# 3dhumangan/3DHumanGAN

Measured on NVIDIA H100. Metric: images_per_sec_G_fwd_512x512, higher is better.
Workload: dtype f32 (bf16x3 split on wgmma, fp32 accumulate)

## Files before the change

### 3dhumangan_b200/csrc/synth.cu

```cuda
#include "common.cuh"
#include "wgmma.cuh"

namespace hg {

constexpr int kC = 256;
constexpr int kSynThreads = 384;
constexpr int kSynStages = 2;
constexpr int kASlots = 2;
constexpr int kXSlots = 5;
constexpr int kXs = 3;
constexpr int kSs = 2;
constexpr uint32_t kAChunk = 128 * 128;
constexpr uint32_t kBStage = 256 * 128;
constexpr uint32_t kXSlice = 32 * 128 * 4;

struct SpadeArgs {
  const float* x;
  long x_bstride;
  const float* mod;
  const float* scsh;
  const float* p_lr;
  long p_stride;
  const float* p_bias;
  const uint8_t* wgb;
  const float* bgb;
  const uint8_t* wimg;
  const float* bias;
  const float* skip;
  long skip_bstride;
  float* out;
  double* stats;
  const float* rgb_w;
  const float* rgb_b;
  const float* rgb_in;
  float* rgb_out;
  int B, HW, Hg, Wg, Rh, Rw;
  int nkc;
  int xC;
  const float* x2;
  float slope;
  int cout;
  int out_pm;
  int act;
  const float* ascale;
  const float* rk_v;
  int rk_n;
  const float* mod2;
};

struct SynSmem {
  uint8_t* a_hi;
  uint8_t* a_lo;
  uint8_t* b_st;
  float* x_st;
  int xs_n, ss_n;
  float* tab_g1;
  float* tab_g0;
  float* tab_bias;
  float* tab_rgbw;
  float* tab_bgb;
  float* tab_as;
  float* st_sum;
  float* st_sq;
  uint64_t* bars;
};

template <bool kPixel>
__device__ __forceinline__ SynSmem carve(uint8_t* raw) {
  constexpr int kA = kPixel ? 3 : kASlots, kX = kPixel ? 3 : kXSlots;
  uint8_t* s = reinterpret_cast<uint8_t*>((reinterpret_cast<uintptr_t>(raw) + 1023) & ~uintptr_t(1023));
  SynSmem m;
  m.a_hi = s;
  m.a_lo = s + kA * kAChunk;
  m.b_st = s + 2 * kA * kAChunk;
  m.x_st = reinterpret_cast<float*>(m.b_st + kSynStages * kBStage);
  m.xs_n = kPixel ? 2 : kXs;
  m.ss_n = kPixel ? 1 : kSs;
  float* f = m.x_st + kX * (kXSlice / 4);
  m.tab_g1 = f; f += kC;
  m.tab_g0 = f; f += kC;
  m.tab_bias = f; f += kC;
  m.tab_rgbw = f; f += 3 * kC;
  m.tab_bgb = f; f += 512;
  m.tab_as = f; f += kC;
  m.st_sum = f; f += kC;
  m.st_sq = f; f += kC;
  m.bars = reinterpret_cast<uint64_t*>(f);
  return m;
}
constexpr uint32_t kSynSmemBytes = 2 * kASlots * kAChunk + kSynStages * kBStage + kXSlots * kXSlice +
                                   (kC * 9 + 512) * 4 + 24 * 8 + 1024;
constexpr uint32_t kPixSmemBytes = 2 * 3 * kAChunk + kSynStages * kBStage + 3 * kXSlice + (kC * 9 + 512) * 4 + 24 * 8 + 1024;
static_assert(kSynSmemBytes <= 232448 && kPixSmemBytes <= 232448, "shared memory budget");

enum { B_FULL = 0 , B_EMPTY = 2 , X_FULL = 4 , X_EMPTY = 12  };

__device__ __forceinline__ void rows_barrier() { named_barrier(1, 256); }

__device__ __forceinline__ float lrelu02(float v) { return v > 0.f ? v : 0.2f * v; }

__device__ __forceinline__ float reduce_2pi(float t) {
  const float y = t * 0.15915494309189535f;
  const float k = (y + 12582912.f) - 12582912.f;
  float r = fmaf(-k, 6.2831854820251465f, t);
  return fmaf(-k, -1.7484555314695172e-07f, r);
}
__device__ __forceinline__ float sin_red(float t) { return __sinf(reduce_2pi(t)); }
__device__ __forceinline__ float cos_red(float t) { return __cosf(reduce_2pi(t)); }
__device__ __forceinline__ float2 reduce_2pi2(float2 t) {
  const float2 y = fmul2(t, make_float2(0.15915494309189535f, 0.15915494309189535f));
  const float2 k = fadd2(fadd2(y, make_float2(12582912.f, 12582912.f)), make_float2(-12582912.f, -12582912.f));
  const float2 r = ffma2(k, make_float2(-6.2831854820251465f, -6.2831854820251465f), t);
  return ffma2(k, make_float2(1.7484555314695172e-07f, 1.7484555314695172e-07f), r);
}
__device__ __forceinline__ float2 sin_red2(float2 t) { const float2 r = reduce_2pi2(t); return make_float2(__sinf(r.x), __sinf(r.y)); }
__device__ __forceinline__ float2 cos_red2(float2 t) { const float2 r = reduce_2pi2(t); return make_float2(__cosf(r.x), __cosf(r.y)); }

struct TileMap {
  int T, first, stride, count;
  __device__ __forceinline__ void get(int it, int& b, int& ti) const {
    const int tile = first + it * stride;
    b = tile / T;
    ti = tile - b * T;
  }
};

__device__ __forceinline__ void init_common(const SpadeArgs& a, const SynSmem& m) {
  for (int i = threadIdx.x; i < kC; i += blockDim.x) {
    m.tab_bias[i] = a.bias[i];
    m.st_sum[i] = 0.f;
    m.st_sq[i] = 0.f;
  }
  if (a.rgb_w)
    for (int i = threadIdx.x; i < 3 * kC; i += blockDim.x) m.tab_rgbw[i] = a.rgb_w[i];
  if (threadIdx.x == 0) {
    for (int i = 0; i < kSynStages; ++i) {
      mbar_init(m.bars + B_FULL + i, 1);
      mbar_init(m.bars + B_EMPTY + i, 2);
    }
    for (int i = 0; i < m.xs_n + m.ss_n; ++i) {
      mbar_init(m.bars + X_FULL + i, 1);
      mbar_init(m.bars + X_EMPTY + i, 8);
    }
    fence_mbar_init();
  }
  __syncthreads();
}

template <int kPasses>
__device__ __forceinline__ void weight_producer_loop(const SynSmem& m, const uint8_t* img, int nstages, int num_my_tiles) {
  uint32_t st = 0, ph = 0;
  for (int t = 0; t < num_my_tiles; ++t)
    for (int s = 0; s < nstages; ++s) {
      if (kPasses == 1 && (s & 1)) continue;
      mbar_wait_backoff(m.bars + B_EMPTY + st, ph ^ 1);
      mbar_arrive_expect_tx(m.bars + B_FULL + st, kBStage);
      bulk_g2s(m.b_st + st * kBStage, img + static_cast<size_t>(s) * kBStage, kBStage, m.bars + B_FULL + st);
      if (++st == kSynStages) { st = 0; ph ^= 1; }
    }
}

struct Pipe {
  uint32_t st = 0, ph = 0, prev = ~0u;
};
template <int N, int kPasses>
__device__ __forceinline__ void pipe_chunk(const SynSmem& m, Pipe& p, float (&d)[N / 2], uint32_t a_hi, uint32_t a_lo, bool accumulate,
                                           int t) {
#pragma unroll
  for (int part = 0; part < (kPasses == 3 ? 2 : 1); ++part) {
    mbar_wait(m.bars + B_FULL + p.st, p.ph);
    acc_fence(d);
    wgmma_fence();
    const uint32_t bt = smem_u32(m.b_st + p.st * kBStage);
    if (part == 0) {
      wg_k64<N>(d, a_hi, bt, accumulate);
      if (kPasses == 3) wg_k64<N>(d, a_lo, bt, true);
    } else {
      wg_k64<N>(d, a_hi, bt, true);
    }
    wgmma_commit();
    wgmma_wait<1>();
    acc_fence(d);
    if (p.prev != ~0u && t == 0) mbar_arrive(m.bars + B_EMPTY + p.prev);
    p.prev = p.st;
    if (++p.st == kSynStages) { p.st = 0; p.ph ^= 1; }
  }
}
template <int N>
__device__ __forceinline__ void pipe_drain(const SynSmem& m, Pipe& p, float (&d)[N / 2], int t) {
  wgmma_wait<0>();
  acc_fence(d);
  if (p.prev != ~0u && t == 0) mbar_arrive(m.bars + B_EMPTY + p.prev);
  p.prev = ~0u;
}

__device__ __forceinline__ void ring_emit(const SynSmem& m, uint32_t& g, int base, int slots, const float* src) {
  const uint32_t slot = base + g % slots;
  mbar_wait_backoff(m.bars + X_EMPTY + slot, ((g / slots) & 1) ^ 1);
  mbar_arrive_expect_tx(m.bars + X_FULL + slot, kXSlice);
  bulk_g2s(m.x_st + slot * (kXSlice / 4), src, kXSlice, m.bars + X_FULL + slot);
  ++g;
}
__device__ __forceinline__ void x_producer_loop(const SpadeArgs& a, const SynSmem& m, const TileMap& tm) {
  uint32_t g = 0;
  for (int it = 0; it < tm.count; ++it) {
    int b, ti;
    tm.get(it, b, ti);
    const int per_src = a.xC / 32;
    const float* base = a.x + static_cast<long>(b) * a.x_bstride + static_cast<long>(ti) * a.xC * 128;
    const float* base2 = a.x2 ? a.x2 + (static_cast<long>(b) * tm.T + ti) * a.xC * 128 : nullptr;
    for (int j = 0; j < 2 * a.nkc; ++j)
      ring_emit(m, g, 0, m.xs_n, (j < per_src ? base : base2 - per_src * 32 * 128) + j * 32 * 128);
  }
}
__device__ __forceinline__ void skip_producer_loop(const SpadeArgs& a, const SynSmem& m, const TileMap& tm) {
  if (!a.skip) return;
  uint32_t g = 0;
  for (int it = 0; it < tm.count; ++it) {
    int b, ti;
    tm.get(it, b, ti);
    const float* base = a.skip + static_cast<long>(b) * a.skip_bstride + static_cast<long>(ti) * a.cout * 128;
    for (int j = 0; j < a.cout / 32; ++j) ring_emit(m, g, m.xs_n, m.ss_n, base + j * 32 * 128);
  }
}

__device__ __forceinline__ uint32_t ring_take(const SynSmem& m, uint32_t g, int base, int slots) {
  const uint32_t slot = base + g % slots;
  mbar_wait_sleep(m.bars + X_FULL + slot, (g / slots) & 1);
  return slot;
}
__device__ __forceinline__ void ring_release(const SynSmem& m, uint32_t slot) {
  __syncwarp();
  if ((threadIdx.x & 31) == 0) mbar_arrive(m.bars + X_EMPTY + slot);
}

__device__ __forceinline__ void take_x_pair(const SynSmem& m, uint32_t& xg, int h, int row, float (&dst)[32]) {
#pragma unroll
  for (int hh = 0; hh < 2; ++hh, ++xg) {
    const uint32_t xslot = ring_take(m, xg, 0, m.xs_n);
    if (hh == h) {
      const uint32_t xs = smem_u32(m.x_st + xslot * (kXSlice / 4)) + row * 4;
#pragma unroll
      for (int j = 0; j < 32; ++j) dst[j] = lds_f32(xs + j * 512);
    }
    ring_release(m, xslot);
  }
}

__device__ __forceinline__ void column_sums(float* st, int c0, const float (&v)[4][2]) {
  const int lane = threadIdx.x & 31, r = lane >> 2;
  const bool b2 = r & 4, b1 = r & 2, b0 = r & 1;
  float w[4], u[2];
#pragma unroll
  for (int i = 0; i < 4; ++i) {
    const float lo = v[i >> 1][i & 1], hi = v[(i + 4) >> 1][i & 1];
    w[i] = (b2 ? hi : lo) + __shfl_xor_sync(0xffffffffu, b2 ? lo : hi, 16);
  }
#pragma unroll
  for (int i = 0; i < 2; ++i)
    u[i] = (b1 ? w[i + 2] : w[i]) + __shfl_xor_sync(0xffffffffu, b1 ? w[i] : w[i + 2], 8);
  const float x = (b0 ? u[1] : u[0]) + __shfl_xor_sync(0xffffffffu, b0 ? u[0] : u[1], 4);
  atomicAdd(st + c0 + 8 * (r >> 1) + 2 * (lane & 3) + (r & 1), x);
}

template <bool kSkip>
__device__ __forceinline__ void epilogue_fwd(const SpadeArgs& a, const SynSmem& m, const float (&d)[128], int b, int ti, int T,
                                             int g, int t, uint32_t& sg) {
  const int HW = a.HW, cout = a.cout;
  const bool kRgb = a.rgb_w != nullptr, kStats = a.stats != nullptr;
  int row[2];
  bool valid[2];
#pragma unroll
  for (int i = 0; i < 2; ++i) {
    row[i] = g * 64 + frag_row(t, i);
    valid[i] = ti * 128 + row[i] < HW;
  }
  float* const otile = a.out + (static_cast<long>(b) * T + ti) * cout * 128;
  float r[2][3] = {{0.f, 0.f, 0.f}, {0.f, 0.f, 0.f}};
#pragma unroll
  for (int cg = 0; cg < 8; ++cg) {
    if (cg * 32 >= cout) break;
    float sk[2][4][2];
    if (kSkip) {
      const uint32_t slot = ring_take(m, sg, m.xs_n, m.ss_n);
      const float* xs = m.x_st + slot * (kXSlice / 4);
#pragma unroll
      for (int i = 0; i < 2; ++i)
#pragma unroll
        for (int jj = 0; jj < 4; ++jj)
#pragma unroll
          for (int e = 0; e < 2; ++e) sk[i][jj][e] = xs[(frag_col(t, jj, e)) * 128 + row[i]];
      ring_release(m, slot);
      ++sg;
    }
    float s1[4][2], s2[4][2];
#pragma unroll
    for (int jj = 0; jj < 4; ++jj)
#pragma unroll
      for (int e = 0; e < 2; ++e) {
        const int j = cg * 4 + jj, c = frag_col(t, j, e);
        const float bc = m.tab_bias[c];
        s1[jj][e] = 0.f;
        s2[jj][e] = 0.f;
#pragma unroll
        for (int i = 0; i < 2; ++i) {
          float v = d[4 * j + 2 * i + e] + bc;
          if (kSkip) v += sk[i][jj][e];
          if (valid[i]) otile[c * 128 + row[i]] = v;
          else v = 0.f;
          if (kRgb) {
#pragma unroll
            for (int k = 0; k < 3; ++k) r[i][k] = fmaf(v, m.tab_rgbw[k * kC + c], r[i][k]);
          }
          s1[jj][e] += v;
          s2[jj][e] = fmaf(v, v, s2[jj][e]);
        }
      }
    if (kStats) {
      column_sums(m.st_sum, cg * 32, s1);
      column_sums(m.st_sq, cg * 32, s2);
    }
  }
  if (kRgb) {
#pragma unroll
    for (int i = 0; i < 2; ++i) {
#pragma unroll
      for (int k = 0; k < 3; ++k) {
        r[i][k] += __shfl_xor_sync(0xffffffffu, r[i][k], 1);
        r[i][k] += __shfl_xor_sync(0xffffffffu, r[i][k], 2);
      }
      if ((t & 3) == 0 && valid[i]) {
        const int pix = ti * 128 + row[i];
#pragma unroll
        for (int k = 0; k < 3; ++k) {
          const long idx = (static_cast<long>(b) * 3 + k) * HW + pix;
          float o = r[i][k] + a.rgb_b[k];
          if (a.rgb_in) o += a.rgb_in[idx];
          a.rgb_out[idx] = o;
        }
      }
    }
  }
}

__device__ __forceinline__ void epilogue_fwd_any(const SpadeArgs& a, const SynSmem& m, const float (&d)[128], int b, int ti, int T,
                                                 int g, int t, uint32_t& sg) {
  if (a.skip) epilogue_fwd<true>(a, m, d, b, ti, T, g, t, sg);
  else epilogue_fwd<false>(a, m, d, b, ti, T, g, t, sg);
}

__device__ __forceinline__ void flush_fwd_stats(const SpadeArgs& a, const SynSmem& m) {
  rows_barrier();
  if (a.stats)
    for (int c = threadIdx.x; c < kC; c += 256) {
      atomicAdd(a.stats + c, static_cast<double>(m.st_sum[c]));
      atomicAdd(a.stats + kC + c, static_cast<double>(m.st_sq[c]));
    }
}

template <bool kSine, bool kRk, bool kPm>
__device__ __forceinline__ void epilogue_bwd(const SpadeArgs& a, const SynSmem& m, const float (&d)[128], int b, int ti, int T, int g,
                                             int t, uint32_t& sg) {
  const int HW = a.HW, cout = a.cout, rk_n = a.rk_n;
  const float mslope = a.slope;
  int row[2];
  bool valid[2];
  float rv[2][3] = {{0.f, 0.f, 0.f}, {0.f, 0.f, 0.f}};
#pragma unroll
  for (int i = 0; i < 2; ++i) {
    row[i] = g * 64 + frag_row(t, i);
    valid[i] = ti * 128 + row[i] < HW;
    if (kRk && valid[i]) {
      const float* rp = a.rk_v + static_cast<long>(b) * rk_n * HW + ti * 128 + row[i];
      rv[i][0] = rp[0];
      if (rk_n > 1) rv[i][1] = rp[HW];
      if (rk_n > 2) rv[i][2] = rp[2 * static_cast<long>(HW)];
    }
  }
  float* const otile = a.out + (static_cast<long>(b) * T + ti) * cout * 128;
#pragma unroll
  for (int cg = 0; cg < 8; ++cg) {
    if (cg * 32 >= cout) break;
    float xv[2][4][2];
    {
      const uint32_t slot = ring_take(m, sg, m.xs_n, m.ss_n);
      const float* xs = m.x_st + slot * (kXSlice / 4);
#pragma unroll
      for (int i = 0; i < 2; ++i)
#pragma unroll
        for (int jj = 0; jj < 4; ++jj)
#pragma unroll
          for (int e = 0; e < 2; ++e)
            xv[i][jj][e] = valid[i] ? xs[frag_col(t, jj, e) * 128 + row[i]] : 0.f;
      ring_release(m, slot);
      ++sg;
    }
    float s1[4][2], s2[4][2];
#pragma unroll
    for (int jj = 0; jj < 4; ++jj)
#pragma unroll
      for (int e = 0; e < 2; ++e) {
        const int j = cg * 4 + jj, c = frag_col(t, j, e);
        const float t1 = m.tab_g1[c], t0 = m.tab_g0[c];
        s1[jj][e] = 0.f;
        s2[jj][e] = 0.f;
#pragma unroll
        for (int i = 0; i < 2; ++i) {
          const float x = xv[i][jj][e];
          const float pre = fmaf(x, t1, t0);
          float acc = d[4 * j + 2 * i + e];
          if (kRk)
            acc = fmaf(rv[i][2], m.tab_rgbw[2 * kC + c], fmaf(rv[i][1], m.tab_rgbw[kC + c], fmaf(rv[i][0], m.tab_rgbw[c], acc)));
          const float mask = kSine ? cos_red(pre) : (pre > 0.f ? 1.f : mslope);
          const float dd = acc * mask;
          if (valid[i]) {
            if (kPm) a.out[(static_cast<long>(b) * HW + ti * 128 + row[i]) * cout + c] = dd;
            else otile[c * 128 + row[i]] = dd;
          }
          s1[jj][e] += dd;
          s2[jj][e] = fmaf(dd, x, s2[jj][e]);
        }
      }
    column_sums(m.st_sum, cg * 32, s1);
    column_sums(m.st_sq, cg * 32, s2);
  }
}

__device__ __forceinline__ void epilogue_bwd_any(const SpadeArgs& a, const SynSmem& m, const float (&d)[128], int b, int ti, int T,
                                                 int g, int t, uint32_t& sg) {
  if (a.act == 1) {
    if (a.rk_v) epilogue_bwd<true, true, false>(a, m, d, b, ti, T, g, t, sg);
    else epilogue_bwd<true, false, false>(a, m, d, b, ti, T, g, t, sg);
  } else {
    if (a.out_pm) epilogue_bwd<false, false, true>(a, m, d, b, ti, T, g, t, sg);
    else epilogue_bwd<false, false, false>(a, m, d, b, ti, T, g, t, sg);
  }
}

__device__ __forceinline__ void flush_bwd_sums(const SpadeArgs& a, const SynSmem& m, int b) {
  for (int c = threadIdx.x; c < a.cout; c += 256) {
    atomicAdd(a.stats + (static_cast<long>(b) * 2 + 0) * a.cout + c, static_cast<double>(m.st_sum[c]));
    atomicAdd(a.stats + (static_cast<long>(b) * 2 + 1) * a.cout + c, static_cast<double>(m.st_sq[c]));
    m.st_sum[c] = 0.f;
    m.st_sq[c] = 0.f;
  }
}

template <int kPasses, bool kBwd>
__global__ void __launch_bounds__(kSynThreads, 1) spade_const_kernel(SpadeArgs a) {
  extern __shared__ uint8_t smem_raw[];
  const SynSmem m = carve<false>(smem_raw);
  const int warp = threadIdx.x >> 5, lane = threadIdx.x & 31;
  init_common(a, m);
  TileMap tm;
  tm.T = (a.HW + 127) / 128;
  tm.first = blockIdx.x;
  tm.stride = gridDim.x;
  tm.count = (a.B * tm.T - static_cast<int>(blockIdx.x) + static_cast<int>(gridDim.x) - 1) / static_cast<int>(gridDim.x);

  if (warp < 8) {
    regs_inc<kMmaRegs>();
    const int g = warp >> 2, t = threadIdx.x & 127;
    const int q = 2 * g + (warp & 1), h = (warp >> 1) & 1;
    const int row = q * 32 + lane;
    int cur_b = -1;
    uint32_t acnt = 0;
    uint32_t xg = 0, sg = 0;
    Pipe p;
    float d[128];
    for (int it = 0; it < tm.count; ++it) {
      int b, ti;
      tm.get(it, b, ti);
      if (b != cur_b) {
        rows_barrier();
        if (kBwd && cur_b >= 0) flush_bwd_sums(a, m, cur_b);
        for (int i = threadIdx.x; i < kC; i += 256) {
          if (kBwd) {
            if (a.ascale) {
              const long ld = a.x2 ? 2 * kC : kC;
              m.tab_as[i] = a.ascale[static_cast<long>(b) * ld + i];
              if (a.x2) m.tab_bgb[i] = a.ascale[static_cast<long>(b) * ld + kC + i];
            }
            if (i < a.cout) {
              m.tab_g1[i] = a.mod ? a.mod[(static_cast<long>(b) * 2 + 0) * a.cout + i] : 1.f;
              m.tab_g0[i] = a.mod ? a.mod[(static_cast<long>(b) * 2 + 1) * a.cout + i] : 0.f;
            }
          } else {
            m.tab_g1[i] = a.mod ? a.mod[(static_cast<long>(b) * 2 + 0) * kC + i] : 1.f;
            m.tab_g0[i] = a.mod ? a.mod[(static_cast<long>(b) * 2 + 1) * kC + i] : 0.f;
            if (a.mod2) {
              m.tab_bgb[i] = a.mod2[(static_cast<long>(b) * 2 + 0) * kC + i];
              m.tab_bgb[kC + i] = a.mod2[(static_cast<long>(b) * 2 + 1) * kC + i];
            }
          }
        }
        rows_barrier();
        cur_b = b;
      }
      const bool valid = ti * 128 + row < a.HW;
      uint32_t tg1a = smem_u32(kBwd ? m.tab_as : m.tab_g1), tg0a = smem_u32(m.tab_g0);
      uint32_t tg1b = smem_u32(m.tab_bgb), tg0b = smem_u32(m.tab_bgb + kC);
      opaque(tg1a);
      opaque(tg0a);
      opaque(tg1b);
      opaque(tg0b);
      const float slope = a.slope;
      const bool sine = a.act == 1, scaled = kBwd && a.ascale != nullptr;
      const bool two_tables = kBwd ? (scaled && a.x2 != nullptr) : a.mod2 != nullptr;
#pragma unroll 1
      for (int kc = 0; kc < a.nkc; ++kc, ++acnt) {
        const int c0 = (kc * 64 + h * 32) & (kC - 1);
        const bool second = two_tables && kc * 64 >= kC;
        const uint32_t tg1 = second ? tg1b : tg1a, tg0 = second ? tg0b : tg0a;
        float cur[32];
        take_x_pair(m, xg, h, row, cur);
        const uint32_t slot = acnt & 1;
#pragma unroll
        for (int gi = 0; gi < 4; ++gi) {
          float y[8], t1[8], t0[8];
          if (!kBwd || scaled) lds8(tg1 + (c0 + gi * 8) * 4, t1);
          if (!kBwd) lds8(tg0 + (c0 + gi * 8) * 4, t0);
          if (kBwd) {
#pragma unroll
            for (int j = 0; j < 8; ++j) y[j] = scaled ? cur[gi * 8 + j] * t1[j] : cur[gi * 8 + j];
          } else if (sine) {
#pragma unroll
            for (int j = 0; j < 8; j += 2) {
              const float2 sv = sin_red2(ffma2(make_float2(cur[gi * 8 + j], cur[gi * 8 + j + 1]), make_float2(t1[j], t1[j + 1]),
                                               make_float2(t0[j], t0[j + 1])));
              y[j] = sv.x;
              y[j + 1] = sv.y;
            }
          } else {
            affine_lrelu8(cur + gi * 8, t1, t0, slope, y);
          }
          if (!valid) {
#pragma unroll
            for (int j = 0; j < 8; ++j) y[j] = 0.f;
          }
          store_a8<kPasses == 3>(m.a_hi + slot * kAChunk, m.a_lo + slot * kAChunk, row, h * 32 + gi * 8, y);
        }
        fence_proxy_async_smem();
        named_barrier(2 + g, 128);
        pipe_chunk<256, kPasses>(m, p, d, smem_u32(m.a_hi + slot * kAChunk) + g * 64 * 128,
                                 smem_u32(m.a_lo + slot * kAChunk) + g * 64 * 128, kc > 0, t);
      }
      pipe_drain<256>(m, p, d, t);
      if (kBwd) epilogue_bwd_any(a, m, d, b, ti, tm.T, g, t, sg);
      else epilogue_fwd_any(a, m, d, b, ti, tm.T, g, t, sg);
    }
    if (kBwd) {
      rows_barrier();
      if (cur_b >= 0) flush_bwd_sums(a, m, cur_b);
    } else {
      flush_fwd_stats(a, m);
    }
  } else {
    regs_dec<kProducerRegs>();
    if (lane == 0) {
      if (warp == 8) weight_producer_loop<kPasses>(m, a.wimg, 2 * a.nkc, tm.count);
      else if (warp == 9) x_producer_loop(a, m, tm);
      else if (warp == 10) skip_producer_loop(a, m, tm);
    }
  }
}

__device__ __forceinline__ void bilin(int dst, int in_size, float scale, int& i0, int& i1, float& l0, float& l1) {
  float src = scale * (static_cast<float>(dst) + 0.5f) - 0.5f;
  src = src < 0.f ? 0.f : src;
  i0 = static_cast<int>(src);
  i1 = i0 + (i0 < in_size - 1 ? 1 : 0);
  l1 = src - static_cast<float>(i0);
  l0 = 1.f - l1;
}

template <int kPasses>
__device__ __forceinline__ void pixel_weight_producer_loop(const SpadeArgs& a, const SynSmem& m, int num_my_tiles) {
  uint32_t st = 0, ph = 0;
  auto emit = [&](const uint8_t* src, uint32_t bytes) {
    mbar_wait_backoff(m.bars + B_EMPTY + st, ph ^ 1);
    mbar_arrive_expect_tx(m.bars + B_FULL + st, bytes);
    bulk_g2s(m.b_st + st * kBStage, src, bytes, m.bars + B_FULL + st);
    if (++st == kSynStages) { st = 0; ph ^= 1; }
  };
  for (int t = 0; t < num_my_tiles; ++t)
    for (int kc = 0; kc < 4; ++kc) {
      for (int k = 0; k < 2; ++k)
        for (int part = 0; part < (kPasses == 3 ? 2 : 1); ++part)
          emit(a.wgb + static_cast<size_t>(((kc >> 1) * 2 + k) * 2 + part) * kBStage + (kc & 1) * (kBStage / 2), kBStage / 2);
      for (int part = 0; part < (kPasses == 3 ? 2 : 1); ++part) emit(a.wimg + static_cast<size_t>(kc * 2 + part) * kBStage, kBStage);
    }
}

template <int kPasses>
__global__ void __launch_bounds__(kSynThreads, 1) spade_pixel_kernel(SpadeArgs a) {
  extern __shared__ uint8_t smem_raw[];
  const SynSmem m = carve<true>(smem_raw);
  const int warp = threadIdx.x >> 5, lane = threadIdx.x & 31;
  for (int i = threadIdx.x; i < kC; i += blockDim.x) {
    m.tab_g1[i] = a.scsh[i];
    m.tab_g0[i] = a.scsh[kC + i];
  }
  for (int i = threadIdx.x; i < 512; i += blockDim.x) m.tab_bgb[i] = a.bgb[i];
  init_common(a, m);
  TileMap tm;
  tm.T = (a.HW + 127) / 128;
  tm.first = blockIdx.x;
  tm.stride = gridDim.x;
  tm.count = (a.B * tm.T - static_cast<int>(blockIdx.x) + static_cast<int>(gridDim.x) - 1) / static_cast<int>(gridDim.x);
  const float sy = static_cast<float>(a.Rh) / static_cast<float>(a.Hg);
  const float sx = static_cast<float>(a.Rw) / static_cast<float>(a.Wg);

  if (warp < 8) {
    regs_inc<kMmaRegs>();
    const int g = warp >> 2, t = threadIdx.x & 127;
    const int q = 2 * g + (warp & 1), h = (warp >> 1) & 1;
    const int row = q * 32 + lane;
    uint8_t* const y_hi = m.a_hi + 2 * kAChunk;
    uint8_t* const y_lo = m.a_lo + 2 * kAChunk;
    uint32_t xg = 0, sg = 0;
    Pipe p;
    float d[128], e[64];
    for (int it = 0; it < tm.count; ++it) {
      int b, ti;
      tm.get(it, b, ti);
      const int pix = ti * 128 + row;
      const bool valid = pix < a.HW;
      {
        const int py = valid ? pix / a.Wg : 0, px = valid ? pix % a.Wg : 0;
        int y0, y1, x0, x1;
        float ly0, ly1, lx0, lx1;
        bilin(py, a.Rh, sy, y0, y1, ly0, ly1);
        bilin(px, a.Rw, sx, x0, x1, lx0, lx1);
        const float* base = a.p_lr + static_cast<long>(b) * a.Rh * a.Rw * a.p_stride;
        const float4* n00 = reinterpret_cast<const float4*>(base + (static_cast<long>(y0) * a.Rw + x0) * a.p_stride);
        const float4* n01 = reinterpret_cast<const float4*>(base + (static_cast<long>(y0) * a.Rw + x1) * a.p_stride);
        const float4* n10 = reinterpret_cast<const float4*>(base + (static_cast<long>(y1) * a.Rw + x0) * a.p_stride);
        const float4* n11 = reinterpret_cast<const float4*>(base + (static_cast<long>(y1) * a.Rw + x1) * a.p_stride);
        const float4* pb = a.p_bias ? reinterpret_cast<const float4*>(a.p_bias + static_cast<long>(b) * 128) : nullptr;
        const float2 lx0p = make_float2(lx0, lx0), lx1p = make_float2(lx1, lx1), ly0p = make_float2(ly0, ly0), ly1p = make_float2(ly1, ly1);
#pragma unroll 2
        for (int gi = 0; gi < 8; ++gi) {
          float y[8];
#pragma unroll
          for (int u = 0; u < 2; ++u) {
            const int f4 = h * 16 + gi * 2 + u;
            const float4 v00 = __ldg(n00 + f4), v01 = __ldg(n01 + f4), v10 = __ldg(n10 + f4), v11 = __ldg(n11 + f4);
            auto lerp2 = [&](float2 a, float2 b, float2 c, float2 d) {
              const float2 top = ffma2(b, lx1p, fmul2(a, lx0p));
              const float2 bot = ffma2(d, lx1p, fmul2(c, lx0p));
              return ffma2(top, ly0p, fmul2(bot, ly1p));
            };
            float2 lo2 = lerp2(make_float2(v00.x, v00.y), make_float2(v01.x, v01.y), make_float2(v10.x, v10.y), make_float2(v11.x, v11.y));
            float2 hi2 = lerp2(make_float2(v00.z, v00.w), make_float2(v01.z, v01.w), make_float2(v10.z, v10.w), make_float2(v11.z, v11.w));
            if (pb) {
              const float4 c4 = __ldg(pb + f4);
              lo2 = fadd2(lo2, make_float2(c4.x, c4.y));
              hi2 = fadd2(hi2, make_float2(c4.z, c4.w));
            }
            y[u * 4 + 0] = lo2.x; y[u * 4 + 1] = lo2.y; y[u * 4 + 2] = hi2.x; y[u * 4 + 3] = hi2.y;
          }
#pragma unroll
          for (int j = 0; j < 8; ++j) y[j] = valid ? fmaxf(y[j], 0.f) : 0.f;
          store_a8<kPasses == 3>(m.a_hi + h * kAChunk, m.a_lo + h * kAChunk, row, gi * 8, y);
        }
        fence_proxy_async_smem();
        named_barrier(2 + g, 128);
      }
      int frow[2];
      bool fvalid[2];
#pragma unroll
      for (int i = 0; i < 2; ++i) {
        frow[i] = g * 64 + frag_row(t, i);
        fvalid[i] = ti * 128 + frow[i] < a.HW;
      }
#pragma unroll 1
      for (int kc = 0; kc < 4; ++kc) {
        for (int k = 0; k < 2; ++k)
          pipe_chunk<128, kPasses>(m, p, e, smem_u32(m.a_hi + k * kAChunk) + g * 64 * 128, smem_u32(m.a_lo + k * kAChunk) + g * 64 * 128,
                                   k > 0, t);
        pipe_drain<128>(m, p, e, t);
        const uint32_t s0 = ring_take(m, xg, 0, m.xs_n), s1 = ring_take(m, xg + 1, 0, m.xs_n);
        xg += 2;
        const float* xs0 = m.x_st + s0 * (kXSlice / 4);
        const float* xs1 = m.x_st + s1 * (kXSlice / 4);
        const int col = (kc >> 1) * 256 + (kc & 1) * 128;
#pragma unroll
        for (int j = 0; j < 8; ++j) {
          const int c = frag_col(t, j, 0), ch = kc * 64 + c;
          const float* xs = j < 4 ? xs0 : xs1;
#pragma unroll
          for (int i = 0; i < 2; ++i) {
            float y2[2];
#pragma unroll
            for (int u = 0; u < 2; ++u) {
              const float gam = e[4 * j + 2 * i + u] + m.tab_bgb[col + c + u];
              const float bet = e[4 * (j + 8) + 2 * i + u] + m.tab_bgb[col + 64 + c + u];
              const float xn = fmaf(xs[((c + u) & 31) * 128 + frow[i]], m.tab_g1[ch + u], m.tab_g0[ch + u]);
              const float v = fmaf(xn, gam, bet);
              y2[u] = fvalid[i] ? fmaxf(v, 0.2f * v) : 0.f;
            }
            uint32_t hb, lb;
            split_bf16x2(y2[0], y2[1], hb, lb);
            const uint32_t off = sw128_offset(frow[i], c);
            asm volatile("st.shared.b32 [%0], %1;" ::"r"(smem_u32(y_hi) + off), "r"(hb));
            if (kPasses == 3) asm volatile("st.shared.b32 [%0], %1;" ::"r"(smem_u32(y_lo) + off), "r"(lb));
          }
        }
        ring_release(m, s0);
        ring_release(m, s1);
        fence_proxy_async_smem();
        named_barrier(2 + g, 128);
        pipe_chunk<256, kPasses>(m, p, d, smem_u32(y_hi) + g * 64 * 128, smem_u32(y_lo) + g * 64 * 128, kc > 0, t);
      }
      pipe_drain<256>(m, p, d, t);
      epilogue_fwd_any(a, m, d, b, ti, tm.T, g, t, sg);
    }
    flush_fwd_stats(a, m);
  } else {
    regs_dec<kProducerRegs>();
    if (lane == 0) {
      if (warp == 8) pixel_weight_producer_loop<kPasses>(a, m, tm.count);
      else if (warp == 9) x_producer_loop(a, m, tm);
      else if (warp == 10) skip_producer_loop(a, m, tm);
    }
  }
}

__global__ void bn_finalize_kernel(const double* __restrict__ stats, double count_in, const double* __restrict__ count_ptr,
                                   const float* __restrict__ weight,
                                   const float* __restrict__ bias, float* running_mean, float* running_var,
                                   int training, float eps, float momentum, const float* __restrict__ gb, int B,
                                   float* __restrict__ scsh, float* __restrict__ mod) {
  const int c = threadIdx.x;
  float mean, var;
  const double count = count_ptr ? count_ptr[0] : count_in;
  if (training) {
    const double mu = stats[c] / count;
    double v = stats[kC + c] / count - mu * mu;
    v = v < 0 ? 0 : v;
    mean = static_cast<float>(mu);
    var = static_cast<float>(v);
    if (running_mean) {
      const double unb = count > 1 ? v * count / (count - 1) : v;
      running_mean[c] = (1.f - momentum) * running_mean[c] + momentum * mean;
      running_var[c] = (1.f - momentum) * running_var[c] + momentum * static_cast<float>(unb);
    }
  } else {
    mean = running_mean[c];
    var = running_var[c];
  }
  const float sc = weight[c] * rsqrtf(var + eps);
  const float sh = bias[c] - mean * sc;
  if (scsh) {
    scsh[c] = sc;
    scsh[kC + c] = sh;
  }
  if (mod && gb) {
    for (int b = 0; b < B; ++b) {
      const float G = gb[(static_cast<long>(b) * 2 + 0) * kC + c];
      const float Bt = gb[(static_cast<long>(b) * 2 + 1) * kC + c];
      mod[(static_cast<long>(b) * 2 + 0) * kC + c] = sc * G;
      mod[(static_cast<long>(b) * 2 + 1) * kC + c] = fmaf(sh, G, Bt);
    }
  }
}

__global__ void synth_input_kernel(const float* __restrict__ w, const float* __restrict__ bias,
                                   const float* __restrict__ ic, const float* __restrict__ jc, int Hg, int Wg,
                                   float* __restrict__ x0, double* __restrict__ stats, double batch_mult) {
  const int c = blockIdx.y;
  const int HW = Hg * Wg;
  const float w0 = w[c * 2 + 0], w1 = w[c * 2 + 1], bb = bias[c];
  float s1 = 0.f, s2 = 0.f;
  for (int p = blockIdx.x * blockDim.x + threadIdx.x; p < HW; p += gridDim.x * blockDim.x) {
    const float v = sinf(fmaf(w1, jc[p % Wg], fmaf(w0, ic[p / Wg], bb)));
    x0[(static_cast<long>(p >> 7) * kC + c) * 128 + (p & 127)] = v;
    s1 += v;
    s2 += v * v;
  }
  __shared__ float r1[8], r2[8];
  for (int o = 16; o > 0; o >>= 1) {
    s1 += __shfl_xor_sync(0xffffffffu, s1, o);
    s2 += __shfl_xor_sync(0xffffffffu, s2, o);
  }
  if ((threadIdx.x & 31) == 0) { r1[threadIdx.x >> 5] = s1; r2[threadIdx.x >> 5] = s2; }
  __syncthreads();
  if (threadIdx.x == 0 && stats) {
    float t1 = 0.f, t2 = 0.f;
    for (int i = 0; i < static_cast<int>(blockDim.x >> 5); ++i) { t1 += r1[i]; t2 += r2[i]; }
    atomicAdd(stats + c, static_cast<double>(t1) * batch_mult);
    atomicAdd(stats + kC + c, static_cast<double>(t2) * batch_mult);
  }
}

}

extern "C" {

int hg_spade_conv(const float* x, long x_bstride, const float* mod, const float* scsh, const float* p_lr,
                  long p_stride, const float* p_bias, const void* wgb, const float* bgb, const void* wimg, const float* bias, const float* skip,
                  float* out, double* stats, const float* rgb_w, const float* rgb_b, const float* rgb_in,
                  float* rgb_out, int B, int C, int Hg, int Wg, int Rh, int Rw, int passes, void* stream) {
  HG_REQUIRE(C == hg::kC, "hg_spade_conv: only %d channels are supported (got %d)", hg::kC, C);
  HG_REQUIRE(x && wimg && bias && out, "hg_spade_conv: null pointer");
  HG_REQUIRE((mod != nullptr) != (p_lr != nullptr), "hg_spade_conv: give exactly one of mod (const style) / p_lr (pixel style)");
  HG_REQUIRE(passes == 1 || passes == 3, "hg_spade_conv: passes must be 1 or 3");
  HG_REQUIRE(B > 0 && Hg > 0 && Wg > 0, "hg_spade_conv: bad shape");
  HG_REQUIRE(!rgb_w || (rgb_b && rgb_out), "hg_spade_conv: rgb_b / rgb_out missing");
  if (p_lr) {
    HG_REQUIRE(scsh && wgb && bgb && Rh > 0 && Rw > 0, "hg_spade_conv: pixel-style arguments missing");
    HG_REQUIRE((reinterpret_cast<uintptr_t>(p_lr) & 15) == 0 && p_stride >= 128 && (p_stride & 3) == 0,
               "hg_spade_conv: p_lr must be 16-byte aligned with a row stride >= 128 that is a multiple of 4");
    HG_REQUIRE(!p_bias || (reinterpret_cast<uintptr_t>(p_bias) & 15) == 0, "hg_spade_conv: p_bias must be 16-byte aligned");
  }
  hg::SpadeArgs a{x, x_bstride, mod, scsh, p_lr, p_stride, p_bias, static_cast<const uint8_t*>(wgb), bgb,
                  static_cast<const uint8_t*>(wimg), bias, skip,
                  static_cast<long>((Hg * Wg + 127) / 128) * hg::kC * 128, out, stats, rgb_w, rgb_b, rgb_in, rgb_out,
                  B, Hg * Wg, Hg, Wg, Rh, Rw};
  a.nkc = 4; a.xC = hg::kC; a.x2 = nullptr; a.slope = 0.2f; a.cout = hg::kC; a.out_pm = 0;
  const int tiles = B * ((Hg * Wg + 127) / 128);
  const int grid = tiles < hg::num_sms() ? tiles : hg::num_sms();
  auto st = static_cast<cudaStream_t>(stream);
#define HG_LAUNCH(KERNEL, SMEM)                                                                                   \
  do {                                                                                                            \
    cudaError_t e = cudaFuncSetAttribute(KERNEL, cudaFuncAttributeMaxDynamicSharedMemorySize, SMEM);               \
    if (e != cudaSuccess) { hg::set_error("hg_spade_conv: smem opt-in failed: %s", cudaGetErrorString(e)); return 2; } \
    KERNEL<<<grid, hg::kSynThreads, SMEM, st>>>(a);                                                               \
  } while (0)
  if (mod) {
    if (passes == 3) HG_LAUNCH((hg::spade_const_kernel<3, false>), hg::kSynSmemBytes); else HG_LAUNCH((hg::spade_const_kernel<1, false>), hg::kSynSmemBytes);
  } else {
    if (passes == 3) HG_LAUNCH(hg::spade_pixel_kernel<3>, hg::kPixSmemBytes); else HG_LAUNCH(hg::spade_pixel_kernel<1>, hg::kPixSmemBytes);
  }
#undef HG_LAUNCH
  return hg::check_launch("hg_spade_conv");
}

static int launch_blocked_gemm(const hg::SpadeArgs& a, int passes, bool bwd, cudaStream_t st, const char* who) {
  const int tiles = a.B * ((a.HW + 127) / 128);
  const int grid = tiles < hg::num_sms() ? tiles : hg::num_sms();
  cudaError_t e;
#define HG_LAUNCH_G(KERNEL)                                                                             \
  do {                                                                                                  \
    e = cudaFuncSetAttribute(KERNEL, cudaFuncAttributeMaxDynamicSharedMemorySize, hg::kSynSmemBytes);   \
    if (e == cudaSuccess) KERNEL<<<grid, hg::kSynThreads, hg::kSynSmemBytes, st>>>(a);                   \
  } while (0)
  if (bwd) {
    if (passes == 3) HG_LAUNCH_G((hg::spade_const_kernel<3, true>)); else HG_LAUNCH_G((hg::spade_const_kernel<1, true>));
  } else {
    if (passes == 3) HG_LAUNCH_G((hg::spade_const_kernel<3, false>)); else HG_LAUNCH_G((hg::spade_const_kernel<1, false>));
  }
#undef HG_LAUNCH_G
  if (e != cudaSuccess) { hg::set_error("%s: smem opt-in failed: %s", who, cudaGetErrorString(e)); return 2; }
  return hg::check_launch(who);
}

int hg_spade_bwd_dgrad(const float* dout, const float* x, long x_bstride, const float* mod, const void* wimg_t, float* dpre,
                       double* sums, int B, int C, int Hg, int Wg, int passes, void* stream) {
  HG_REQUIRE(C == hg::kC, "hg_spade_bwd_dgrad: only %d channels are supported (got %d)", hg::kC, C);
  HG_REQUIRE(dout && x && mod && wimg_t && dpre && sums, "hg_spade_bwd_dgrad: null pointer");
  HG_REQUIRE(passes == 1 || passes == 3, "hg_spade_bwd_dgrad: passes must be 1 or 3");
  HG_REQUIRE(B > 0 && Hg > 0 && Wg > 0, "hg_spade_bwd_dgrad: bad shape");
  const long T = (Hg * Wg + 127) / 128;
  hg::SpadeArgs a{};
  a.x = dout;
  a.x_bstride = T * hg::kC * 128;
  a.mod = mod;
  a.wimg = static_cast<const uint8_t*>(wimg_t);
  a.bias = mod;
  a.skip = x;
  a.skip_bstride = x_bstride;
  a.out = dpre;
  a.stats = sums;
  a.B = B; a.HW = Hg * Wg; a.Hg = Hg; a.Wg = Wg;
  a.nkc = 4; a.xC = hg::kC; a.slope = 0.2f; a.cout = hg::kC;
  return launch_blocked_gemm(a, passes, true, static_cast<cudaStream_t>(stream), "hg_spade_bwd_dgrad");
}

int hg_conv1x1_blocked(const float* x, int Cin, const void* wimg, const float* bias, float* out, int B, int Hg, int Wg,
                       int passes, void* stream) {
  HG_REQUIRE(x && wimg && bias && out, "hg_conv1x1_blocked: null pointer");
  HG_REQUIRE(Cin == 64 || Cin == 128 || Cin == 256, "hg_conv1x1_blocked: Cin must be 64, 128 or 256 (got %d)", Cin);
  HG_REQUIRE(passes == 1 || passes == 3, "hg_conv1x1_blocked: passes must be 1 or 3");
  HG_REQUIRE(B > 0 && Hg > 0 && Wg > 0, "hg_conv1x1_blocked: bad shape");
  const long T = (Hg * Wg + 127) / 128;
  hg::SpadeArgs a{};
  a.x = x;
  a.x_bstride = T * Cin * 128;
  a.wimg = static_cast<const uint8_t*>(wimg);
  a.bias = bias;
  a.skip_bstride = T * hg::kC * 128;
  a.out = out;
  a.B = B; a.HW = Hg * Wg; a.Hg = Hg; a.Wg = Wg;
  a.nkc = Cin / 64; a.xC = Cin; a.slope = 1.f; a.cout = hg::kC;
  return launch_blocked_gemm(a, passes, false, static_cast<cudaStream_t>(stream), "hg_conv1x1_blocked");
}

int hg_act_conv1x1_blocked(const float* x, const float* x2, const float* mod, int act, const void* wimg, const float* bias,
                           float* out, int B, int Hg, int Wg, int passes, void* stream) {
  HG_REQUIRE(x && mod && wimg && bias && out, "hg_act_conv1x1_blocked: null pointer");
  HG_REQUIRE(act == 0 || act == 1, "hg_act_conv1x1_blocked: act must be 0 (LeakyReLU 0.2) or 1 (sine)");
  HG_REQUIRE(passes == 1 || passes == 3, "hg_act_conv1x1_blocked: passes must be 1 or 3");
  HG_REQUIRE(B > 0 && Hg > 0 && Wg > 0, "hg_act_conv1x1_blocked: bad shape");
  const long T = (Hg * Wg + 127) / 128;
  hg::SpadeArgs a{};
  a.x = x;
  a.x_bstride = T * hg::kC * 128;
  a.x2 = x2;
  a.mod = mod;
  a.wimg = static_cast<const uint8_t*>(wimg);
  a.bias = bias;
  a.skip_bstride = T * hg::kC * 128;
  a.out = out;
  a.B = B; a.HW = Hg * Wg; a.Hg = Hg; a.Wg = Wg;
  a.nkc = x2 ? 8 : 4; a.xC = hg::kC; a.slope = 0.2f; a.cout = hg::kC; a.act = act;
  return launch_blocked_gemm(a, passes, false, static_cast<cudaStream_t>(stream), "hg_act_conv1x1_blocked");
}

int hg_blocked_conv_wide(const float* x, const float* x2, const float* mod, const float* mod2, int act, float slope,
                         const void* wimg, const float* bias, const float* skip, float* out, double* stats,
                         const float* rgb_w, const float* rgb_b, const float* rgb_in, float* rgb_out, int B, int Hg, int Wg,
                         int passes, void* stream) {
  HG_REQUIRE(x && wimg && bias && out, "hg_blocked_conv_wide: null pointer");
  HG_REQUIRE(act == 0 || act == 1, "hg_blocked_conv_wide: act must be 0 (LeakyReLU(slope)) or 1 (sine)");
  HG_REQUIRE(!mod2 || (mod && x2), "hg_blocked_conv_wide: mod2 needs mod and a second source");
  HG_REQUIRE(!rgb_w || (rgb_b && rgb_out), "hg_blocked_conv_wide: rgb_b / rgb_out missing");
  HG_REQUIRE(passes == 1 || passes == 3, "hg_blocked_conv_wide: passes must be 1 or 3");
  HG_REQUIRE(B > 0 && Hg > 0 && Wg > 0, "hg_blocked_conv_wide: bad shape");
  const long T = (Hg * Wg + 127) / 128;
  hg::SpadeArgs a{};
  a.x = x;
  a.x_bstride = T * hg::kC * 128;
  a.x2 = x2;
  a.mod = mod;
  a.mod2 = mod2;
  a.wimg = static_cast<const uint8_t*>(wimg);
  a.bias = bias;
  a.skip = skip;
  a.skip_bstride = T * hg::kC * 128;
  a.out = out;
  a.stats = stats;
  a.rgb_w = rgb_w; a.rgb_b = rgb_b; a.rgb_in = rgb_in; a.rgb_out = rgb_out;
  a.B = B; a.HW = Hg * Wg; a.Hg = Hg; a.Wg = Wg;
  a.nkc = x2 ? 8 : 4; a.xC = hg::kC; a.slope = slope; a.cout = hg::kC; a.act = act;
  return launch_blocked_gemm(a, passes, false, static_cast<cudaStream_t>(stream), "hg_blocked_conv_wide");
}

int hg_conv1x1_blocked_bwd(const float* g, const float* g2, const float* aux, const float* mod, const void* wimg_t,
                           float* out, double* sums, int Cout, float slope, int pixel_major, int act, const float* ascale,
                           const float* rk_w, const float* rk_v, int rk_n, int B, int Hg, int Wg, int passes,
                           void* stream) {
  HG_REQUIRE(act == 0 || act == 1, "hg_conv1x1_blocked_bwd: act must be 0 (LeakyReLU/ReLU mask) or 1 (cosine)");
  HG_REQUIRE(!rk_v || (rk_w && rk_n >= 1 && rk_n <= 3 && Cout == 256), "hg_conv1x1_blocked_bwd: bad rank-k term");
  HG_REQUIRE(g && aux && wimg_t && out && sums, "hg_conv1x1_blocked_bwd: null pointer");
  HG_REQUIRE(Cout == 128 || Cout == 256, "hg_conv1x1_blocked_bwd: Cout must be 128 or 256 (got %d)", Cout);
  HG_REQUIRE(!pixel_major || Cout == 128, "hg_conv1x1_blocked_bwd: the pixel-major output is built for Cout == 128");
  HG_REQUIRE(!(act == 1 && pixel_major) && !(act == 0 && rk_v),
             "hg_conv1x1_blocked_bwd: compiled epilogues are sine [+ rank-k term] / LeakyReLU [+ pixel-major output]");
  HG_REQUIRE(passes == 1 || passes == 3, "hg_conv1x1_blocked_bwd: passes must be 1 or 3");
  HG_REQUIRE(B > 0 && Hg > 0 && Wg > 0, "hg_conv1x1_blocked_bwd: bad shape");
  const long T = (Hg * Wg + 127) / 128;
  hg::SpadeArgs a{};
  a.x = g;
  a.x_bstride = T * hg::kC * 128;
  a.x2 = g2;
  a.mod = mod;
  a.wimg = static_cast<const uint8_t*>(wimg_t);
  a.bias = static_cast<const float*>(wimg_t);
  a.skip = aux;
  a.skip_bstride = T * Cout * 128;
  a.out = out;
  a.stats = sums;
  a.B = B; a.HW = Hg * Wg; a.Hg = Hg; a.Wg = Wg;
  a.nkc = g2 ? 8 : 4; a.xC = hg::kC; a.slope = slope; a.cout = Cout; a.out_pm = pixel_major;
  a.act = act; a.ascale = ascale; a.rgb_w = rk_v ? rk_w : nullptr; a.rk_v = rk_v; a.rk_n = rk_n;
  return launch_blocked_gemm(a, passes, true, static_cast<cudaStream_t>(stream), "hg_conv1x1_blocked_bwd");
}

int hg_bn_finalize(const double* stats, double count, const double* count_dev, const float* weight, const float* bias, float* running_mean,
                   float* running_var, int training, float eps, float momentum, const float* gb, int B, int C,
                   float* scsh, float* mod, void* stream) {
  HG_REQUIRE(C == hg::kC, "hg_bn_finalize: only %d channels are supported (got %d)", hg::kC, C);
  HG_REQUIRE(weight && bias && (scsh || mod), "hg_bn_finalize: null pointer");
  HG_REQUIRE(training ? (stats != nullptr && (count > 0 || count_dev)) : (running_mean && running_var),
             "hg_bn_finalize: statistics missing");
  hg::bn_finalize_kernel<<<1, hg::kC, 0, static_cast<cudaStream_t>(stream)>>>(
      stats, count, count_dev, weight, bias, running_mean, running_var, training, eps, momentum, gb, B, scsh, mod);
  return hg::check_launch("hg_bn_finalize");
}

int hg_synth_input(const float* w, const float* bias, const float* ic, const float* jc, int C, int Hg, int Wg,
                   float* x0, double* stats, int batch, void* stream) {
  HG_REQUIRE(C == hg::kC, "hg_synth_input: only %d channels are supported (got %d)", hg::kC, C);
  HG_REQUIRE(w && bias && ic && jc && x0, "hg_synth_input: null pointer");
  const int HW = Hg * Wg;
  int bx = (HW + 255) / 256;
  if (bx > 32) bx = 32;
  dim3 grid(bx, C);
  hg::synth_input_kernel<<<grid, 256, 0, static_cast<cudaStream_t>(stream)>>>(w, bias, ic, jc, Hg, Wg, x0, stats,
                                                                              static_cast<double>(batch));
  return hg::check_launch("hg_synth_input");
}

}
```

Measured before the change: 100.0.

## Split weight pipeline stages into half-width chunks with four-deep ring

The weight staging ring now uses four half-size (N=128) stages instead of two full-size stages. The producer issues two half copies per former stage, and the consumer runs wgmma on each N-half separately with its own barrier wait. The goal is finer-grained overlap of weight bulk copies with tensor-core work at the same shared-memory footprint. In exchange it adds more barrier waits, commits and wgmma_wait<1> points, and the pixel kernel consumers must still match the new half-stage granularity.

```diff
diff --git a/3dhumangan_b200/csrc/synth.cu b/3dhumangan_b200/csrc/synth.cu
--- a/3dhumangan_b200/csrc/synth.cu
+++ b/3dhumangan_b200/csrc/synth.cu
@@ -5,13 +5,14 @@
 
 constexpr int kC = 256;
 constexpr int kSynThreads = 384;
-constexpr int kSynStages = 2;
+constexpr int kHStages = 4;
 constexpr int kASlots = 2;
 constexpr int kXSlots = 5;
 constexpr int kXs = 3;
 constexpr int kSs = 2;
 constexpr uint32_t kAChunk = 128 * 128;
 constexpr uint32_t kBStage = 256 * 128;
+constexpr uint32_t kBHalf = kBStage / 2;
 constexpr uint32_t kXSlice = 32 * 128 * 4;
 
 struct SpadeArgs {
@@ -73,7 +74,7 @@
   m.a_hi = s;
   m.a_lo = s + kA * kAChunk;
   m.b_st = s + 2 * kA * kAChunk;
-  m.x_st = reinterpret_cast<float*>(m.b_st + kSynStages * kBStage);
+  m.x_st = reinterpret_cast<float*>(m.b_st + kHStages * kBHalf);
   m.xs_n = kPixel ? 2 : kXs;
   m.ss_n = kPixel ? 1 : kSs;
   float* f = m.x_st + kX * (kXSlice / 4);
@@ -88,12 +89,12 @@
   m.bars = reinterpret_cast<uint64_t*>(f);
   return m;
 }
-constexpr uint32_t kSynSmemBytes = 2 * kASlots * kAChunk + kSynStages * kBStage + kXSlots * kXSlice +
+constexpr uint32_t kSynSmemBytes = 2 * kASlots * kAChunk + kHStages * kBHalf + kXSlots * kXSlice +
                                    (kC * 9 + 512) * 4 + 24 * 8 + 1024;
-constexpr uint32_t kPixSmemBytes = 2 * 3 * kAChunk + kSynStages * kBStage + 3 * kXSlice + (kC * 9 + 512) * 4 + 24 * 8 + 1024;
+constexpr uint32_t kPixSmemBytes = 2 * 3 * kAChunk + kHStages * kBHalf + 3 * kXSlice + (kC * 9 + 512) * 4 + 24 * 8 + 1024;
 static_assert(kSynSmemBytes <= 232448 && kPixSmemBytes <= 232448, "shared memory budget");
 
-enum { B_FULL = 0 , B_EMPTY = 2 , X_FULL = 4 , X_EMPTY = 12  };
+enum { B_FULL = 0 , B_EMPTY = 4 , X_FULL = 8 , X_EMPTY = 16  };
 
 __device__ __forceinline__ void rows_barrier() { named_barrier(1, 256); }
 
@@ -134,7 +135,7 @@
   if (a.rgb_w)
     for (int i = threadIdx.x; i < 3 * kC; i += blockDim.x) m.tab_rgbw[i] = a.rgb_w[i];
   if (threadIdx.x == 0) {
-    for (int i = 0; i < kSynStages; ++i) {
+    for (int i = 0; i < kHStages; ++i) {
       mbar_init(m.bars + B_FULL + i, 1);
       mbar_init(m.bars + B_EMPTY + i, 2);
     }
@@ -153,10 +154,12 @@
   for (int t = 0; t < num_my_tiles; ++t)
     for (int s = 0; s < nstages; ++s) {
       if (kPasses == 1 && (s & 1)) continue;
-      mbar_wait_backoff(m.bars + B_EMPTY + st, ph ^ 1);
-      mbar_arrive_expect_tx(m.bars + B_FULL + st, kBStage);
-      bulk_g2s(m.b_st + st * kBStage, img + static_cast<size_t>(s) * kBStage, kBStage, m.bars + B_FULL + st);
-      if (++st == kSynStages) { st = 0; ph ^= 1; }
+      for (int n = 0; n < 2; ++n) {
+        mbar_wait_backoff(m.bars + B_EMPTY + st, ph ^ 1);
+        mbar_arrive_expect_tx(m.bars + B_FULL + st, kBHalf);
+        bulk_g2s(m.b_st + st * kBHalf, img + static_cast<size_t>(s) * kBStage + n * kBHalf, kBHalf, m.bars + B_FULL + st);
+        if (++st == kHStages) { st = 0; ph ^= 1; }
+      }
     }
 }
 
@@ -167,24 +170,27 @@
 __device__ __forceinline__ void pipe_chunk(const SynSmem& m, Pipe& p, float (&d)[N / 2], uint32_t a_hi, uint32_t a_lo, bool accumulate,
                                            int t) {
 #pragma unroll
-  for (int part = 0; part < (kPasses == 3 ? 2 : 1); ++part) {
-    mbar_wait(m.bars + B_FULL + p.st, p.ph);
-    acc_fence(d);
-    wgmma_fence();
-    const uint32_t bt = smem_u32(m.b_st + p.st * kBStage);
-    if (part == 0) {
-      wg_k64<N>(d, a_hi, bt, accumulate);
-      if (kPasses == 3) wg_k64<N>(d, a_lo, bt, true);
-    } else {
-      wg_k64<N>(d, a_hi, bt, true);
-    }
-    wgmma_commit();
-    wgmma_wait<1>();
-    acc_fence(d);
-    if (p.prev != ~0u && t == 0) mbar_arrive(m.bars + B_EMPTY + p.prev);
-    p.prev = p.st;
-    if (++p.st == kSynStages) { p.st = 0; p.ph ^= 1; }
-  }
+  for (int part = 0; part < (kPasses == 3 ? 2 : 1); ++part)
+#pragma unroll
+    for (int n = 0; n < N / 128; ++n) {
+      float (&dn)[64] = *reinterpret_cast<float(*)[64]>(d + 64 * n);
+      mbar_wait(m.bars + B_FULL + p.st, p.ph);
+      acc_fence(d);
+      wgmma_fence();
+      const uint32_t bt = smem_u32(m.b_st + p.st * kBHalf);
+      if (part == 0) {
+        wg_k64<128>(dn, a_hi, bt, accumulate);
+        if (kPasses == 3) wg_k64<128>(dn, a_lo, bt, true);
+      } else {
+        wg_k64<128>(dn, a_hi, bt, true);
+      }
+      wgmma_commit();
+      wgmma_wait<1>();
+      acc_fence(d);
+      if (p.prev != ~0u && t == 0) mbar_arrive(m.bars + B_EMPTY + p.prev);
+      p.prev = p.st;
+      if (++p.st == kHStages) { p.st = 0; p.ph ^= 1; }
+    }
 }
 template <int N>
 __device__ __forceinline__ void pipe_drain(const SynSmem& m, Pipe& p, float (&d)[N / 2], int t) {
@@ -577,18 +583,19 @@
 template <int kPasses>
 __device__ __forceinline__ void pixel_weight_producer_loop(const SpadeArgs& a, const SynSmem& m, int num_my_tiles) {
   uint32_t st = 0, ph = 0;
-  auto emit = [&](const uint8_t* src, uint32_t bytes) {
+  auto emit = [&](const uint8_t* src) {
     mbar_wait_backoff(m.bars + B_EMPTY + st, ph ^ 1);
-    mbar_arrive_expect_tx(m.bars + B_FULL + st, bytes);
-    bulk_g2s(m.b_st + st * kBStage, src, bytes, m.bars + B_FULL + st);
-    if (++st == kSynStages) { st = 0; ph ^= 1; }
+    mbar_arrive_expect_tx(m.bars + B_FULL + st, kBHalf);
+    bulk_g2s(m.b_st + st * kBHalf, src, kBHalf, m.bars + B_FULL + st);
+    if (++st == kHStages) { st = 0; ph ^= 1; }
   };
   for (int t = 0; t < num_my_tiles; ++t)
     for (int kc = 0; kc < 4; ++kc) {
       for (int k = 0; k < 2; ++k)
         for (int part = 0; part < (kPasses == 3 ? 2 : 1); ++part)
-          emit(a.wgb + static_cast<size_t>(((kc >> 1) * 2 + k) * 2 + part) * kBStage + (kc & 1) * (kBStage / 2), kBStage / 2);
-      for (int part = 0; part < (kPasses == 3 ? 2 : 1); ++part) emit(a.wimg + static_cast<size_t>(kc * 2 + part) * kBStage, kBStage);
+          emit(a.wgb + static_cast<size_t>(((kc >> 1) * 2 + k) * 2 + part) * kBStage + (kc & 1) * kBHalf);
+      for (int part = 0; part < (kPasses == 3 ? 2 : 1); ++part)
+        for (int n = 0; n < 2; ++n) emit(a.wimg + static_cast<size_t>(kc * 2 + part) * kBStage + n * kBHalf);
     }
 }
 
```

Result: faster. 103.7 (median of 6 runs) (+3.7%).
